# ygtxr1997/CelebBasis

Hardware: NVIDIA H100
Metric: celeb-basis training steps/sec (SD-v1 UNet 512^2, bs=1/GPU) (higher is better)
Workload: dtype f16 operands / f32 accumulate+residual (reference: f32 with TF32 convs)

## Files before the change

### celebbasis_b200/csrc/cb_attention.cu

```cuda
#include <string.h>

#include <type_traits>

#include "cb_common.cuh"

namespace cb {

constexpr int kAttnConsumers = 256;
constexpr int kAttnThreads = kAttnConsumers + 128;
constexpr int kAttnProducerRegs = 24;
constexpr int kAttnConsumerRegs = 240;
constexpr int kBQ = 128;
constexpr int kBKV = 64;

struct AttnParams {
    int nq, nk, heads, images;
    int d;
    int causal;
    int two_pass;
    float scale_log2e;
    void* O;
    long long ldo;
    float* lse;
    void* P;
    long long ldp;
    int is_bf16;
};

template <int DBOX>
struct AttnCfg {
    static constexpr int kQBytes = DBOX * kBQ * 128;
    static constexpr int kKBytes = DBOX * kBKV * 128;
    static constexpr int kVBytes = DBOX * kBKV * 128;
    static constexpr int kPBytes = kBQ * 128;
    static constexpr int kStages = 4;
    static constexpr int kSmemBytes = kQBytes + kStages * (kKBytes + kVBytes) + 2 * kPBytes + 1024 + 256;
};

__device__ __forceinline__ void mbar_wait_consumer(uint32_t bar, uint32_t parity) {
    while (!mbar_try_wait(bar, parity)) {
    }
}

template <uint32_t R>
__device__ __forceinline__ void regs_dealloc() { asm volatile("setmaxnreg.dec.sync.aligned.u32 %0;" ::"n"(R)); }
template <uint32_t R>
__device__ __forceinline__ void regs_alloc() { asm volatile("setmaxnreg.inc.sync.aligned.u32 %0;" ::"n"(R)); }

template <int KS, bool BF16>
__device__ __forceinline__ void mma_rows(float (&acc)[32], uint32_t a, uint32_t a_box, uint32_t b, uint32_t b_box) {
    wgmma_fence();
#pragma unroll
    for (int k = 0; k < KS; ++k)
        Wgmma<64, BF16, 0, 0>::mma(acc, gmma_desc_sw128(a + (k >> 2) * a_box + (k & 3) * 32, 16, 1024),
                                   gmma_desc_sw128(b + (k >> 2) * b_box + (k & 3) * 32, 16, 1024), k > 0 ? 1u : 0u);
    wgmma_commit();
}
template <int KS>
__device__ __forceinline__ void mma_rows_any(bool bf16, float (&acc)[32], uint32_t a, uint32_t a_box, uint32_t b,
                                             uint32_t b_box) {
    if (bf16) mma_rows<KS, true>(acc, a, a_box, b, b_box);
    else mma_rows<KS, false>(acc, a, a_box, b, b_box);
}
template <int NO, bool BF16>
__device__ __forceinline__ void mma_block(float (&acc)[NO / 2], uint32_t a, uint32_t y, uint32_t acc_in) {
    wgmma_fence();
#pragma unroll
    for (int k = 0; k < kBKV / 16; ++k)
        Wgmma<NO, BF16, 0, 1>::mma(acc, gmma_desc_sw128(a + k * 32, 16, 1024), gmma_desc_sw128(y + k * 2048, kBKV * 128, 1024),
                                   k > 0 ? 1u : acc_in);
    wgmma_commit();
}
template <int NO>
__device__ __forceinline__ void mma_block_any(bool bf16, float (&acc)[NO / 2], uint32_t a, uint32_t y, uint32_t acc_in) {
    if (bf16) mma_block<NO, true>(acc, a, y, acc_in);
    else mma_block<NO, false>(acc, a, y, acc_in);
}

__device__ __forceinline__ float fast_exp2(float x) {
    float y;
    asm("ex2.approx.ftz.f32 %0, %1;" : "=f"(y) : "f"(x));
    return y;
}
__device__ __forceinline__ uint32_t pack2(float a, float b, bool bf16) {
    if (bf16) {
        __nv_bfloat162 h = __floats2bfloat162_rn(a, b);
        return *reinterpret_cast<uint32_t*>(&h);
    }
    __half2 h = __floats2half2_rn(a, b);
    return *reinterpret_cast<uint32_t*>(&h);
}
__device__ __forceinline__ void st_a_pair(uint32_t tile, int r, int col, uint32_t v) {
    const uint32_t dst = tile + r * 128 + ((((uint32_t)col >> 3) ^ ((uint32_t)r & 7u)) << 4) + (col & 7) * 2;
    asm volatile("st.shared.b32 [%0], %1;" ::"r"(dst), "r"(v) : "memory");
}
__device__ __forceinline__ float quad_max(float v) {
    v = fmaxf(v, __shfl_xor_sync(0xffffffffu, v, 1));
    return fmaxf(v, __shfl_xor_sync(0xffffffffu, v, 2));
}
__device__ __forceinline__ float quad_sum(float v) {
    v += __shfl_xor_sync(0xffffffffu, v, 1);
    return v + __shfl_xor_sync(0xffffffffu, v, 2);
}

template <int KS>
__global__ void __launch_bounds__(kAttnThreads, 1)
cb_attention_fwd_kernel(const __grid_constant__ CUtensorMap tmQ, const __grid_constant__ CUtensorMap tmK,
                        const __grid_constant__ CUtensorMap tmV, const __grid_constant__ AttnParams p) {
    constexpr int DBOX = (KS + 3) / 4;
    using Cfg = AttnCfg<DBOX>;
    constexpr int kSt = Cfg::kStages;
    constexpr int NO = DBOX * 64;
    extern __shared__ uint8_t smem_raw[];
    const uint32_t base = (smem_u32(smem_raw) + 1023u) & ~1023u;
    const uint32_t sQ = base;
    const uint32_t sKV = sQ + Cfg::kQBytes;
    const uint32_t sP = sKV + kSt * (Cfg::kKBytes + Cfg::kVBytes);
    const uint32_t bars = sP + 2 * Cfg::kPBytes;
    const uint32_t bar_q = bars;
    auto bar_kv_full = [&](int s) { return bars + 8u * (1 + s); };
    auto bar_kv_empty = [&](int s) { return bars + 8u * (1 + kSt + s); };

    const int warp = threadIdx.x >> 5, lane = threadIdx.x & 31;
    const int wg = __shfl_sync(0xffffffffu, warp >> 2, 0);
    const int q0 = blockIdx.x * kBQ;
// ... 659 lines not shown
```

### celebbasis_b200/csrc/cb_common.cuh

```cuda
#pragma once

#include <cuda.h>
#include <cuda_fp16.h>
#include <cuda_bf16.h>
#include <cuda_runtime.h>
#include <stdint.h>

#include "../../include/celebbasis_b200.h"
#include "cb_wgmma.cuh"

namespace cb {

void set_error(const char* fmt, ...);
int  check_cuda(cudaError_t e, const char* what);

#define CB_REQUIRE(cond, code, ...)                      \
    do {                                                 \
        if (!(cond)) {                                   \
            ::cb::set_error(__VA_ARGS__);                \
            return (code);                               \
        }                                                \
    } while (0)

#define CB_CUDA(call)                                                 \
// ... 35 lines not shown
                                                cudaStream_t st, Args&&... args) {
    cudaLaunchConfig_t cfg = {};
    cfg.gridDim = grid;
    cfg.blockDim = block;
    cfg.dynamicSmemBytes = smem;
    cfg.stream = st;
    cudaLaunchAttribute at[2];
    at[0].id = cudaLaunchAttributeClusterDimension;
    at[0].val.clusterDim.x = cluster.x;
    at[0].val.clusterDim.y = cluster.y;
    at[0].val.clusterDim.z = cluster.z;
    at[1].id = cudaLaunchAttributeProgrammaticStreamSerialization;
    at[1].val.programmaticStreamSerializationAllowed = 1;
    cfg.attrs = at;
    cfg.numAttrs = pdl_enabled() ? 2 : 1;
    return cudaLaunchKernelEx(&cfg, kern, static_cast<KArgs>(args)...);
}
#define CB_LAUNCH(kern, grid, block, smem, st, ...) \
    ::cb::launch_kernel(kern, dim3(grid), dim3(block), (size_t)(smem), (st), ##__VA_ARGS__)
#endif

#if defined(__CUDACC__)

__device__ __forceinline__ uint32_t smem_u32(const void* p) {
    return static_cast<uint32_t>(__cvta_generic_to_shared(p));
}

__device__ __forceinline__ uint32_t lane_id() { return threadIdx.x & 31u; }

__device__ __forceinline__ void pdl_launch_dependents() { asm volatile("griddepcontrol.launch_dependents;" ::: "memory"); }
__device__ __forceinline__ void pdl_wait() { asm volatile("griddepcontrol.wait;" ::: "memory"); }
__device__ __forceinline__ void pdl_sync() {
    pdl_launch_dependents();
    pdl_wait();
}

__device__ __forceinline__ bool elect_one() {
    uint32_t pred = 0;
    asm volatile(
        "{\n"
        ".reg .pred P;\n"
        "elect.sync _|P, 0xffffffff;\n"
        "selp.u32 %0, 1, 0, P;\n"
        "}\n"
        : "=r"(pred));
    return pred != 0;
}

__device__ __forceinline__ void mbar_init(uint32_t bar, uint32_t count) {
    asm volatile("mbarrier.init.shared::cta.b64 [%0], %1;" ::"r"(bar), "r"(count));
}
__device__ __forceinline__ void mbar_fence_init() {
    asm volatile("fence.mbarrier_init.release.cluster;" ::: "memory");
}
__device__ __forceinline__ void fence_proxy_async_smem() {
    asm volatile("fence.proxy.async.shared::cta;" ::: "memory");
}
__device__ __forceinline__ void mbar_arrive_expect_tx(uint32_t bar, uint32_t bytes) {
    asm volatile("mbarrier.arrive.expect_tx.shared::cta.b64 _, [%0], %1;" ::"r"(bar), "r"(bytes)
                 : "memory");
}
__device__ __forceinline__ void mbar_arrive(uint32_t bar) {
    asm volatile("mbarrier.arrive.shared::cta.b64 _, [%0];" ::"r"(bar) : "memory");
}
__device__ __forceinline__ bool mbar_try_wait(uint32_t bar, uint32_t parity) {
    uint32_t ok;
    asm volatile(
        "{\n"
        ".reg .pred P;\n"
        "mbarrier.try_wait.parity.shared::cta.b64 P, [%1], %2;\n"
        "selp.u32 %0, 1, 0, P;\n"
        "}\n"
        : "=r"(ok)
        : "r"(bar), "r"(parity)
        : "memory");
    return ok != 0;
}
__device__ __forceinline__ void mbar_wait(uint32_t bar, uint32_t parity) {
    uint32_t spins = 0;
    while (!mbar_try_wait(bar, parity)) {
        if (++spins > (1u << 26)) __trap();
    }
}

__device__ __forceinline__ void tma_prefetch_desc(const CUtensorMap* m) {
    asm volatile("prefetch.tensormap [%0];" ::"l"(reinterpret_cast<uint64_t>(m)) : "memory");
}
__device__ __forceinline__ void tma_load_2d(uint32_t dst, const CUtensorMap* m, uint32_t bar, int c0,
                                            int c1) {
    asm volatile(
        "cp.async.bulk.tensor.2d.shared::cluster.global.mbarrier::complete_tx::bytes [%0], [%1, {%3, %4}], "
        "[%2];" ::"r"(dst),
        "l"(reinterpret_cast<uint64_t>(m)), "r"(bar), "r"(c0), "r"(c1)
        : "memory");
}
__device__ __forceinline__ void tma_load_3d(uint32_t dst, const CUtensorMap* m, uint32_t bar, int c0,
                                            int c1, int c2) {
    asm volatile(
        "cp.async.bulk.tensor.3d.shared::cluster.global.mbarrier::complete_tx::bytes [%0], [%1, {%3, %4, "
        "%5}], [%2];" ::"r"(dst),
        "l"(reinterpret_cast<uint64_t>(m)), "r"(bar), "r"(c0), "r"(c1), "r"(c2)
        : "memory");
}
__device__ __forceinline__ void tma_load_4d(uint32_t dst, const CUtensorMap* m, uint32_t bar, int c0,
                                            int c1, int c2, int c3) {
    asm volatile(
        "cp.async.bulk.tensor.4d.shared::cluster.global.mbarrier::complete_tx::bytes [%0], [%1, {%3, %4, "
        "%5, %6}], [%2];" ::"r"(dst),
        "l"(reinterpret_cast<uint64_t>(m)), "r"(bar), "r"(c0), "r"(c1), "r"(c2), "r"(c3)
        : "memory");
}

__device__ __forceinline__ void tma_bulk_g2s(uint32_t dst, const void* src, uint32_t bytes, uint32_t bar) {
    asm volatile("cp.async.bulk.shared::cluster.global.mbarrier::complete_tx::bytes [%0], [%1], %2, [%3];" ::"r"(dst),
                 "l"(reinterpret_cast<uint64_t>(src)), "r"(bytes), "r"(bar)
                 : "memory");
}

__device__ __forceinline__ void wgmma_fence() { asm volatile("wgmma.fence.sync.aligned;" ::: "memory"); }
__device__ __forceinline__ void wgmma_commit() { asm volatile("wgmma.commit_group.sync.aligned;" ::: "memory"); }
template <int N>
__device__ __forceinline__ void wgmma_wait() { asm volatile("wgmma.wait_group.sync.aligned %0;" ::"n"(N) : "memory"); }
template <int R>
__device__ __forceinline__ void wgmma_fence_regs(float (&d)[R]) {
#pragma unroll
    for (int i = 0; i < R; ++i) asm volatile("" : "+f"(d[i])::"memory");
}
__device__ __forceinline__ void named_bar(int id, int n) { asm volatile("bar.sync %0, %1;" ::"r"(id), "r"(n) : "memory"); }

__device__ __forceinline__ uint32_t cluster_ctarank() {
    uint32_t r;
    asm volatile("mov.u32 %0, %%cluster_ctarank;" : "=r"(r));
    return r;
}
__device__ __forceinline__ void cluster_sync_all() {
    asm volatile("barrier.cluster.arrive.release.aligned;\n\tbarrier.cluster.wait.acquire.aligned;" ::: "memory");
}

__device__ __forceinline__ void st_cluster_f32x8(uint32_t addr, uint32_t cta, const uint32_t* v) {
    asm volatile(
        "{\n"
        ".reg .b32 ra;\n"
        "mapa.shared::cluster.u32 ra, %0, %1;\n"
        "st.shared::cluster.v4.b32 [ra], {%2, %3, %4, %5};\n"
        "st.shared::cluster.v4.b32 [ra + 16], {%6, %7, %8, %9};\n"
        "}\n" ::"r"(addr),
        "r"(cta), "r"(v[0]), "r"(v[1]), "r"(v[2]), "r"(v[3]), "r"(v[4]), "r"(v[5]), "r"(v[6]), "r"(v[7])
        : "memory");
}
__device__ __forceinline__ void st_cluster_f32x2(uint32_t addr, uint32_t cta, float a, float b) {
    asm volatile(
        "{\n"
        ".reg .b32 ra;\n"
        "mapa.shared::cluster.u32 ra, %0, %1;\n"
        "st.shared::cluster.v2.f32 [ra], {%2, %3};\n"
        "}\n" ::"r"(addr),
        "r"(cta), "f"(a), "f"(b)
        : "memory");
}
__device__ __forceinline__ void cluster_arrive_relaxed() { asm volatile("barrier.cluster.arrive.relaxed.aligned;" ::: "memory"); }
__device__ __forceinline__ void cluster_wait() { asm volatile("barrier.cluster.wait.acquire.aligned;" ::: "memory"); }
__device__ __forceinline__ float4 ld_shared_f32x4(uint32_t addr) {
    float4 v;
    asm volatile("ld.shared.v4.f32 {%0, %1, %2, %3}, [%4];" : "=f"(v.x), "=f"(v.y), "=f"(v.z), "=f"(v.w) : "r"(addr) : "memory");
    return v;
}
// ... 43 lines not shown
```

### celebbasis_b200/csrc/cb_gemm.cu

```cuda
#include <algorithm>
#include <stdarg.h>
#include <stdio.h>
#include <stdlib.h>
#include <string.h>

#include "cb_common.cuh"

namespace cb {

constexpr int BM = 128;
constexpr int BK = 64;
constexpr int kThreads = 384;

struct GemmParams {
    int M, N, K;
    int kchunks, taps, kw;
    int ksteps_last;
    int conv;
    int out_h, out_w, img_n;
    int box_w, box_h, box_i;
    int tiles_w, tiles_h;
    int stride, pad_top, pad_left;
    int b_tap_rows, flip_taps;
    void* D;
    int d_dtype;
    long long ldd, d_bs, d_bs2;
    void* D2;
    int d2_dtype;
    long long ldd2;
    int glu;
    const float* act_param;
    const float* d2_scale;
    const float* d2_shift;
    int batch_inner;
    int d_transposed;
    int vec_ok;
    int force_stages;
    const float* bias;
    int bias_row_div;
    long long ldbias;
    const void* R;
    int r_dtype;
    long long ldr, r_bs, r_bs2;
    float alpha;
    int act;
    int bf16;
    unsigned a_bytes, b_bytes;
    int splits, kiters_per_split;
    float* ws;
    unsigned* counters;
    int cluster_sk;
    int dbg_mode;
    unsigned long long* dbg;
};

template <int BN, int kStages>
struct TileCfg {
    static constexpr int kTmemCols = BN <= 64 ? 64 : (BN <= 128 ? 128 : 256);
    static constexpr int kABytes = BM * BK * 2;
    static constexpr int kBBytes = BN * BK * 2;
    static constexpr int kStageBytes = kABytes + kBBytes;
    static constexpr int kSmemBytes = kStages * kStageBytes + 1024 + 256;
    static_assert(kStages * kStageBytes >= BM * (BN + 4) * 4, "the accumulator tile is staged in the TMA ring");
};

__device__ __forceinline__ unsigned long long gtimer() {
    unsigned long long t;
    asm volatile("mov.u64 %0, %globaltimer;" : "=l"(t));
    return t;
}

__device__ __forceinline__ float apply_act(float v, int act) {
    switch (act) {
        case CB_ACT_SILU: return silu_f(v);
        case CB_ACT_GELU: return gelu_f(v);
        case CB_ACT_QUICK_GELU: return quick_gelu_f(v);
        default: return v;
    }
}

__device__ __forceinline__ void apply_act8(float (&f)[8], int act, const float* act_param, int col, int ncols = 8) {
    if (act == CB_ACT_PRELU) {
#pragma unroll
        for (int j = 0; j < 8; ++j)
            if (j < ncols) f[j] = f[j] > 0.f ? f[j] : f[j] * __ldg(act_param + col + j);
    } else {
#pragma unroll
        for (int j = 0; j < 8; ++j) f[j] = apply_act(f[j], act);
    }
}
__device__ __forceinline__ void d2_affine8(float (&g)[8], const float (&f)[8], const float* sc, const float* sh, int col,
                                           int ncols = 8) {
#pragma unroll
    for (int j = 0; j < 8; ++j) g[j] = (sc && j < ncols) ? f[j] * __ldg(sc + col + j) + __ldg(sh + col + j) : f[j];
}

template <typename T>
__device__ __forceinline__ void load8(const T* p, float (&f)[8]);
template <>
__device__ __forceinline__ void load8<__half>(const __half* p, float (&f)[8]) {
    uint4 u = *reinterpret_cast<const uint4*>(p);
    const __half2* h = reinterpret_cast<const __half2*>(&u);
#pragma unroll
    for (int i = 0; i < 4; ++i) {
        float2 t = __half22float2(h[i]);
        f[2 * i] = t.x;
        f[2 * i + 1] = t.y;
    }
}
template <>
__device__ __forceinline__ void load8<__nv_bfloat16>(const __nv_bfloat16* p, float (&f)[8]) {
    uint4 u = *reinterpret_cast<const uint4*>(p);
    const __nv_bfloat162* h = reinterpret_cast<const __nv_bfloat162*>(&u);
#pragma unroll
    for (int i = 0; i < 4; ++i) {
        float2 t = __bfloat1622float2(h[i]);
        f[2 * i] = t.x;
        f[2 * i + 1] = t.y;
    }
}
template <>
__device__ __forceinline__ void load8<float>(const float* p, float (&f)[8]) {
    float4 a = *reinterpret_cast<const float4*>(p);
    float4 b = *reinterpret_cast<const float4*>(p + 4);
    f[0] = a.x; f[1] = a.y; f[2] = a.z; f[3] = a.w;
    f[4] = b.x; f[5] = b.y; f[6] = b.z; f[7] = b.w;
}

template <typename T>
__device__ __forceinline__ void store8(T* p, const float (&f)[8]);
template <>
__device__ __forceinline__ void store8<__half>(__half* p, const float (&f)[8]) {
    uint4 u;
    __half2* h = reinterpret_cast<__half2*>(&u);
#pragma unroll
    for (int i = 0; i < 4; ++i) h[i] = __floats2half2_rn(f[2 * i], f[2 * i + 1]);
    *reinterpret_cast<uint4*>(p) = u;
}
template <>
__device__ __forceinline__ void store8<__nv_bfloat16>(__nv_bfloat16* p, const float (&f)[8]) {
    uint4 u;
    __nv_bfloat162* h = reinterpret_cast<__nv_bfloat162*>(&u);
#pragma unroll
    for (int i = 0; i < 4; ++i) h[i] = __floats2bfloat162_rn(f[2 * i], f[2 * i + 1]);
    *reinterpret_cast<uint4*>(p) = u;
}
template <>
// ... 234 lines not shown
            float f[8] = {0.f, 0.f, 0.f, 0.f, 0.f, 0.f, 0.f, 0.f};
#pragma unroll 4
            for (int s2 = 0; s2 < S; ++s2) {
                const uint32_t a = xbuf + static_cast<uint32_t>(((s2 * GI + gi) * BM + row) * 32);
                const float4 lo = ld_shared_f32x4(a), hi = ld_shared_f32x4(a + 16);
                f[0] += lo.x; f[1] += lo.y; f[2] += lo.z; f[3] += lo.w;
                f[4] += hi.x; f[5] += hi.y; f[6] += hi.z; f[7] += hi.w;
            }
#pragma unroll
            for (int j = 0; j < 8; ++j) f[j] *= p.alpha;
            epilogue_group8<kExt>(p, f, grow, s_brow[row], n0 + g * 8, d_off, r_off, min(8, ncols_tile - g * 8), nullptr,
                                  sbias_of(row, g * 8));
        }
        return;
    }

    if constexpr (kExt) {
        if (p.glu) {
            constexpr int GQ = BN / 16;
#pragma unroll 1
            for (int u = tid; u < BM * GQ; u += kThreads) {
                const int row = u / GQ, q = u % GQ;
                const int vcol = (q >> 2) * 64 + (q & 3) * 8;
                const long long grow = s_grow[row];
                if (vcol >= ncols_tile || grow < 0) continue;
                float fv[8], fg[8];
                stage_ld8(stage + row * kPitch + vcol, p.alpha, fv);
                stage_ld8(stage + row * kPitch + vcol + 32, p.alpha, fg);
#pragma unroll
                for (int j = 0; j < 8; ++j) {
                    fv[j] += p.bias ? s_bias[vcol + j] : 0.f;
                    fg[j] += p.bias ? s_bias[vcol + 32 + j] : 0.f;
                }
                if (p.D) {
                    store8_any(p.D, p.d_dtype, grow * p.ldd + n0 + vcol, fv);
                    store8_any(p.D, p.d_dtype, grow * p.ldd + n0 + vcol + 32, fg);
                }
                float h[8];
#pragma unroll
                for (int j = 0; j < 8; ++j) h[j] = fv[j] * gelu_f(fg[j]);
                store8_any(p.D2, p.d2_dtype, grow * p.ldd2 + ((n0 + (q >> 2) * 64) >> 1) + (q & 3) * 8, h);
            }
            return;
        }
    }

    const bool r_pre = p.R && p.vec_ok && !p.d_transposed;
    uint4 rq[kResAhead + 1][2];
    auto res_fetch = [&](int k, uint4 (&v)[2]) {
        const int u = tid + k * kThreads;
        if (u >= BM * G) return;
        const int row = u / G, col = (u % G) * 8;
        const long long grow = s_grow[row];
        if (grow >= 0 && col + 8 <= ncols_tile) residual_load8(p, r_off + grow * p.ldr + n0 + col, v);
    };
    if (r_pre) {
#pragma unroll
        for (int k = 0; k < kResAhead; ++k) res_fetch(k, rq[k]);
    }
    const int nunits = (BM * G - tid + kThreads - 1) / kThreads;
#pragma unroll 1
    for (int k = 0; k < nunits; ++k) {
        if (r_pre) res_fetch(k + kResAhead, rq[kResAhead]);
        const int u = tid + k * kThreads;
        const int row = p.d_transposed ? u % BM : u / G;
        const int col = (p.d_transposed ? u / BM : u % G) * 8;
        const long long grow = s_grow[row];
        if (col < ncols_tile && grow >= 0) {
            const int ncols = min(8, ncols_tile - col);
            float f[8], r[8];
            stage_ld8(stage + row * kPitch + col, p.alpha, f);
            if (r_pre && ncols == 8) residual_unpack8(p, rq[0], r);
            epilogue_group8<kExt>(p, f, grow, s_brow[row], n0 + col, d_off, r_off, ncols, r_pre && ncols == 8 ? r : nullptr,
                                  sbias_of(row, col));
        }
        if (dbg && k == 0 && tid == 64) dbg[6] = clock64();
        if (r_pre) {
#pragma unroll
            for (int j = 0; j < kResAhead; ++j) { rq[j][0] = rq[j + 1][0]; rq[j][1] = rq[j + 1][1]; }
        }
    }
}

template <int BN, bool A_MN, bool B_MN, int kStages, bool kExt>
__global__ void __launch_bounds__(kThreads, 1)
cb_gemm_kernel(const __grid_constant__ CUtensorMap tmA, const __grid_constant__ CUtensorMap tmB,
               const __grid_constant__ GemmParams p) {
    using Cfg = TileCfg<BN, kStages>;
    using SCfg = StageCfg<BN>;
    extern __shared__ uint8_t smem_raw[];
    const uint32_t smem_base = (smem_u32(smem_raw) + 1023u) & ~1023u;
    float* stage = reinterpret_cast<float*>(smem_raw + (smem_base - smem_u32(smem_raw)));
    const uint32_t bar_base = smem_base + kStages * Cfg::kStageBytes;
    auto full_bar = [&](int s) { return bar_base + 8u * s; };
    auto empty_bar = [&](int s) { return bar_base + 8u * (kStages + s); };

    __shared__ long long s_grow[BM];
    __shared__ int s_brow[BM];
    __shared__ __align__(16) float s_bias[BN];
    const int warp = threadIdx.x >> 5;
    const int wg = __shfl_sync(0xffffffffu, warp >> 2, 0);
    if (p.dbg_mode == 3) { pdl_sync(); return; }
    unsigned long long* dbg = p.dbg ? p.dbg + 8ull * ((blockIdx.z * gridDim.y + blockIdx.y) * gridDim.x + blockIdx.x) : nullptr;
    if (dbg && threadIdx.x == 0) { dbg[0] = clock64(); dbg[7] = gtimer(); }
    const int n0 = blockIdx.x * BN;
    const int m_tile = blockIdx.y;
    const int sp = blockIdx.z % p.splits;
    const int bz = blockIdx.z / p.splits;
    const int zi = bz % p.batch_inner;
    const int zo = bz / p.batch_inner;

    int m0 = 0, ow0 = 0, oh0 = 0, img0 = 0;
    if (p.conv) {
        const int tw = m_tile % p.tiles_w;
        const int th = (m_tile / p.tiles_w) % p.tiles_h;
        const int ti = m_tile / (p.tiles_w * p.tiles_h);
        ow0 = tw * p.box_w;
        oh0 = th * p.box_h;
        img0 = ti * p.box_i;
    } else {
        m0 = m_tile * BM;
    }

    if (threadIdx.x == 0) {
        tma_prefetch_desc(&tmA);
        tma_prefetch_desc(&tmB);
        for (int s = 0; s < kStages; ++s) {
            mbar_init(full_bar(s), 1);
            mbar_init(empty_bar(s), 8);
        }
        mbar_fence_init();
        fence_proxy_async_smem();
    }
    __syncthreads();
    if (dbg && threadIdx.x == 0) dbg[1] = clock64();
    pdl_sync();

    const int kiters_all = p.dbg_mode == 1 ? 0 : p.taps * p.kchunks;
    const int it0 = sp * p.kiters_per_split;
    const int it1 = min(kiters_all, it0 + p.kiters_per_split);

    if (wg == 0) {
        if (threadIdx.x == 0) {
            int s = 0;
            uint32_t ph = 0;
            int tap = it0 / p.kchunks;
            int kc = it0 - tap * p.kchunks;
            int r = tap / p.kw;
            int sx = tap - r * p.kw;
            for (int it = it0; it < it1; ++it) {
                mbar_wait(empty_bar(s), ph ^ 1u);
                mbar_arrive_expect_tx(full_bar(s), p.a_bytes + p.b_bytes);
                const uint32_t a_dst = smem_base + s * Cfg::kStageBytes;
                const uint32_t b_dst = a_dst + Cfg::kABytes;
                const int tap_b = p.flip_taps ? (p.taps - 1 - tap) : tap;
                if (p.conv) {
                    tma_load_4d(a_dst, &tmA, full_bar(s), kc * BK, ow0 * p.stride + sx - p.pad_left,
                                oh0 * p.stride + r - p.pad_top, img0);
                } else if (A_MN) {
                    tma_load_4d(a_dst, &tmA, full_bar(s), m0, kc * BK, zi, zo);
                    tma_load_4d(a_dst + 8192, &tmA, full_bar(s), m0 + 64, kc * BK, zi, zo);
                } else {
                    tma_load_4d(a_dst, &tmA, full_bar(s), kc * BK, m0, zi, zo);
                }
                if (B_MN) {
#pragma unroll
                    for (int j = 0; j < BN / 64; ++j)
                        tma_load_4d(b_dst + j * 8192, &tmB, full_bar(s), n0 + j * 64,
                                    tap_b * p.b_tap_rows + kc * BK, zi, zo);
                } else {
                    tma_load_4d(b_dst, &tmB, full_bar(s), kc * BK, tap_b * p.b_tap_rows + n0, zi, zo);
                }
                if (++s == kStages) { s = 0; ph ^= 1u; }
                if (++kc == p.kchunks) {
                    kc = 0;
                    ++tap;
                    if (++sx == p.kw) { sx = 0; ++r; }
                }
            }
        }
        __syncwarp();
        const int r = threadIdx.x;
        long long grow;
        bool row_valid;
        if (p.conv) {
            const int per_img = p.box_h * p.box_w;
            const int bi = r / per_img;
            const int rem = r - bi * per_img;
            const int bh = rem / p.box_w;
            const int bw = rem - bh * p.box_w;
            const int img = img0 + bi, oh = oh0 + bh, ow = ow0 + bw;
            row_valid = (bi < p.box_i) && (img < p.img_n) && (oh < p.out_h) && (ow < p.out_w);
            grow = ((long long)img * p.out_h + oh) * p.out_w + ow;
        } else {
            grow = m0 + r;
            row_valid = grow < p.M;
        }
        s_grow[r] = row_valid ? grow : -1;
        if (p.bias) {
            const long long tile_row0 = p.conv ? (((long long)img0 * p.out_h + oh0) * p.out_w + ow0) : (long long)m0;
            const long long brow0 = p.bias_row_div > 0 ? tile_row0 / p.bias_row_div : 0;
            const long long brow = p.bias_row_div > 0 ? grow / p.bias_row_div : 0;
            s_brow[r] = brow == brow0 ? -1 : static_cast<int>(brow);
            const int ncols = min(BN, p.N - n0);
            for (int i = r; i < BN; i += 128) s_bias[i] = i < ncols ? p.bias[brow0 * p.ldbias + n0 + i] : 0.f;
        }
    } else {
        float acc[BN / 2];
#pragma unroll
        for (int i = 0; i < BN / 2; ++i) acc[i] = 0.f;
        const uint32_t a_half = static_cast<uint32_t>(wg - 1) * 8192u;
        const bool releaser = (threadIdx.x & 31) == 0;
        int s = 0, s_prev = 0;
        uint32_t ph = 0;
        int kc = it0 % p.kchunks;
        for (int it = it0; it < it1; ++it) {
            mbar_wait(full_bar(s), ph);
            if (dbg && it == it0 && threadIdx.x == 128) dbg[2] = clock64();
            const uint32_t a_src = smem_base + s * Cfg::kStageBytes + a_half;
            const uint32_t b_src = smem_base + s * Cfg::kStageBytes + Cfg::kABytes;
            const int ksteps = (kc == p.kchunks - 1) ? p.ksteps_last : (BK / 16);
            wgmma_fence_regs(acc);
            if (p.bf16) mma_kiter<BN, A_MN, B_MN, true>(acc, a_src, b_src, ksteps);
            else mma_kiter<BN, A_MN, B_MN, false>(acc, a_src, b_src, ksteps);
            wgmma_wait<1>();
            wgmma_fence_regs(acc);
            if (it > it0 && releaser) mbar_arrive(empty_bar(s_prev));
            s_prev = s;
            if (++s == kStages) { s = 0; ph ^= 1u; }
            if (++kc == p.kchunks) kc = 0;
        }
        wgmma_wait<0>();
        wgmma_fence_regs(acc);
        if (it1 > it0 && releaser) mbar_arrive(empty_bar(s_prev));
        if (dbg && threadIdx.x == 128) dbg[3] = clock64();
        named_bar(4, 256);
        const int l = threadIdx.x & 31, w = warp & 3;
        float* srow = stage + ((wg - 1) * 64 + w * 16 + (l >> 2)) * SCfg::kPitch + 2 * (l & 3);
#pragma unroll
        for (int j = 0; j < BN / 8; ++j) {
            *reinterpret_cast<float2*>(srow + 8 * j) = make_float2(acc[4 * j], acc[4 * j + 1]);
            *reinterpret_cast<float2*>(srow + 8 * SCfg::kPitch + 8 * j) = make_float2(acc[4 * j + 2], acc[4 * j + 3]);
        }
    }
    named_bar(2, kThreads);
    const int ncols_tile = min(BN, p.N - n0);
    if (p.splits > 1 && !p.cluster_sk && p.dbg_mode == 0) {
        const unsigned tile_id = (static_cast<unsigned>(bz) * gridDim.y + m_tile) * gridDim.x + blockIdx.x;
        if (!splitk_reduce_to_stage<BN>(p, tile_id, sp, stage, ncols_tile)) return;
    }
    if (p.dbg_mode == 1 || p.dbg_mode == 2) return;
    if (dbg && threadIdx.x == 64) dbg[4] = clock64();
    epilogue_units<BN, kExt>(p, stage, s_grow, s_brow, s_bias, n0, ncols_tile, zo, zi, sp, smem_base + SCfg::kBytes, dbg);
    if (dbg && threadIdx.x == 64) dbg[5] = clock64();
}

typedef CUresult (*EncodeTiledFn)(CUtensorMap*, CUtensorMapDataType, cuuint32_t, void*, const cuuint64_t*,
                                  const cuuint64_t*, const cuuint32_t*, const cuuint32_t*,
                                  CUtensorMapInterleave, CUtensorMapSwizzle, CUtensorMapL2promotion,
                                  CUtensorMapFloatOOBfill);

static EncodeTiledFn get_encode_fn() {
    static EncodeTiledFn fn = nullptr;
    static bool tried = false;
    if (!tried) {
        tried = true;
        void* p = nullptr;
        cudaDriverEntryPointQueryResult q;
        if (cudaGetDriverEntryPoint("cuTensorMapEncodeTiled", &p, cudaEnableDefault, &q) == cudaSuccess &&
            q == cudaDriverEntryPointSuccess) {
            fn = reinterpret_cast<EncodeTiledFn>(p);
        }
    }
    return fn;
}

int make_tmap(CUtensorMap* out, int dtype, int rank, const void* ptr, const uint64_t* dims,
              const uint64_t* strides_bytes , const uint32_t* box, const uint32_t* estr) {
    EncodeTiledFn fn = get_encode_fn();
    CB_REQUIRE(fn != nullptr, CB_ERR_DRIVER, "cuTensorMapEncodeTiled entry point unavailable");
    CB_REQUIRE((reinterpret_cast<uintptr_t>(ptr) & 15u) == 0, CB_ERR_ALIGN, "tensor base %p not 16B aligned", ptr);
    for (int i = 0; i < rank - 1; ++i)
        CB_REQUIRE((strides_bytes[i] & 15u) == 0, CB_ERR_ALIGN, "tensor stride[%d]=%llu bytes not multiple of 16", i,
                   (unsigned long long)strides_bytes[i]);
    CUtensorMapDataType dt = dtype == CB_F16 ? CU_TENSOR_MAP_DATA_TYPE_FLOAT16 : CU_TENSOR_MAP_DATA_TYPE_BFLOAT16;
    CUresult rc = fn(out, dt, (cuuint32_t)rank, const_cast<void*>(ptr), dims, strides_bytes, box, estr,
                     CU_TENSOR_MAP_INTERLEAVE_NONE, CU_TENSOR_MAP_SWIZZLE_128B, CU_TENSOR_MAP_L2_PROMOTION_L2_256B,
                     CU_TENSOR_MAP_FLOAT_OOB_FILL_NONE);
    CB_REQUIRE(rc == CUDA_SUCCESS, CB_ERR_DRIVER,
               "cuTensorMapEncodeTiled failed rc=%d rank=%d dims=[%llu,%llu,%llu,%llu] box=[%u,%u,%u,%u]", (int)rc,
               rank, (unsigned long long)dims[0], (unsigned long long)dims[1],
               (unsigned long long)(rank > 2 ? dims[2] : 0), (unsigned long long)(rank > 3 ? dims[3] : 0), box[0],
               box[1], rank > 2 ? box[2] : 0, rank > 3 ? box[3] : 0);
    return 0;
}

static inline bool needs_ext(const GemmParams& p) { return p.D2 != nullptr || p.act == CB_ACT_PRELU || p.glu; }

template <int BN, bool A_MN, bool B_MN, int kStages, bool kExt>
static int launch_se(const CUtensorMap& tA, const CUtensorMap& tB, const GemmParams& p, dim3 grid, cudaStream_t st) {
    using Cfg = TileCfg<BN, kStages>;
    static bool attr_done = false;
    auto kern = cb_gemm_kernel<BN, A_MN, B_MN, kStages, kExt>;
    if (!attr_done) {
        CB_CUDA(cudaFuncSetAttribute(kern, cudaFuncAttributeMaxDynamicSharedMemorySize, Cfg::kSmemBytes));
        attr_done = true;
    }
    if (p.cluster_sk) {
        const int S = p.splits;
        CB_REQUIRE(S >= 2 && S <= 16 && grid.z % S == 0, CB_ERR_ARG, "cb_gemm(cluster split-K): %d slices not in [2,16]", S);
        static bool np_done = false;
        if (S > 8 && !np_done) {
            CB_CUDA(cudaFuncSetAttribute(kern, cudaFuncAttributeNonPortableClusterSizeAllowed, 1));
            np_done = true;
        }
        CB_CUDA(launch_kernel_cluster(kern, grid, dim3(kThreads), dim3(1, 1, (unsigned)S), (size_t)Cfg::kSmemBytes, st, tA, tB, p));
        CB_CUDA(cudaGetLastError());
        count_launches(1);
        return 0;
    }
CB_LAUNCH((kern), grid, kThreads, Cfg::kSmemBytes, st, tA, tB, p);
    CB_CUDA(cudaGetLastError());
    count_launches(1);
    return 0;
}

template <int BN, bool A_MN, bool B_MN, int kStages>
static int launch_s(const CUtensorMap& tA, const CUtensorMap& tB, const GemmParams& p, dim3 grid, cudaStream_t st) {
    return needs_ext(p) ? launch_se<BN, A_MN, B_MN, kStages, true>(tA, tB, p, grid, st)
                        : launch_se<BN, A_MN, B_MN, kStages, false>(tA, tB, p, grid, st);
}

static int ring_stages(int bn, const GemmParams& p, long long ctas) {
    if (bn == 256) return 4;
    static const int env_force = getenv("CB_GEMM_STAGES") ? atoi(getenv("CB_GEMM_STAGES")) : 0;
    const int force = p.force_stages ? p.force_stages : env_force;
    if (force == 3) return 3;
    if (force == 6 || ctas <= device_sm_count()) return 6;
    return 3;
}
static bool cluster_sk_fits(int bn, int splits, int stages) {
    const long long stage_bytes = ((long long)BM * (bn + 4) * 4 + 1023) / 1024 * 1024;
    const long long ring = (long long)stages * (BM * BK * 2 + bn * BK * 2);
    const long long gi = (bn / 8 + splits - 1) / splits;
    return stage_bytes + (long long)splits * gi * BM * 32 <= ring;
}

template <int BN, bool A_MN, bool B_MN>
static int launch(const CUtensorMap& tA, const CUtensorMap& tB, const GemmParams& p, dim3 grid, cudaStream_t st) {
    if constexpr (BN == 256) {
        return launch_s<BN, A_MN, B_MN, 4>(tA, tB, p, grid, st);
    } else {
        const long long ctas = (long long)grid.x * grid.y * grid.z;
        if (ring_stages(BN, p, ctas) == 6) return launch_s<BN, A_MN, B_MN, 6>(tA, tB, p, grid, st);
        return launch_s<BN, A_MN, B_MN, 3>(tA, tB, p, grid, st);
    }
}

static double tile_time_us(int bn, long long tiles, int kiters, int sms) {
    const double t_iter = (128.0 + bn) * 128.0 / 80e3;
    const long long waves = (tiles + sms - 1) / sms;
    return (double)waves * kiters * t_iter;
}

static int pick_bn(const cb_gemm_desc& d, int m_tiles, int kiters, bool requested = true) {
    const int N = d.N;
    const int sms = device_sm_count();
    int cands[3];
    int nc = 0;
    if (d.b_major == CB_MAJOR_MN) {
        if (N <= 64) return 64;
        cands[nc++] = 128;
        cands[nc++] = 64;
    } else {
        if (N <= 64) return 64;
        cands[nc++] = 160;
        cands[nc++] = 128;
        cands[nc++] = 64;
    }
    static const int env_bn = getenv("CB_GEMM_BN") ? atoi(getenv("CB_GEMM_BN")) : 0;
    const int force_bn = !requested ? 0 : (d.tile_n > 0 ? d.tile_n : env_bn);
    if (force_bn == 256 && N >= 256) return 256;
    for (int i = 0; i < nc; ++i)
        if (cands[i] == force_bn) return force_bn;
    int best = cands[0];
    double best_t = 1e30;
    for (int i = 0; i < nc; ++i) {
        const int bn = cands[i];
        const long long tiles = (long long)ceil_div(N, bn) * m_tiles * d.batch;
        double t = tile_time_us(bn, tiles, kiters, sms) + 0.02 * ceil_div(N, bn);
        if (t < best_t) { best_t = t; best = bn; }
    }
    return best;
}

}

using namespace cb;

extern "C" int cb_gemm(const cb_gemm_desc* dp, void* stream) {
    CB_REQUIRE(dp != nullptr, CB_ERR_ARG, "cb_gemm: null desc");
    const cb_gemm_desc& d = *dp;
    CB_REQUIRE(d.ab_dtype == CB_F16 || d.ab_dtype == CB_BF16, CB_ERR_ARG, "cb_gemm: ab_dtype must be f16/bf16");
    CB_REQUIRE(d.A && d.B && (d.D || (d.glu && d.D2)), CB_ERR_ARG, "cb_gemm: null A/B/D");
    if (d.glu) {
        CB_REQUIRE(d.D2 && d.N % 64 == 0 && d.batch == 1 && !d.d_transposed && !d.R && d.act == CB_ACT_NONE &&
                       d.bias_row_div == 0,
                   CB_ERR_ARG, "cb_gemm(glu): needs D2, N %% 64 == 0, batch 1, no residual / activation / per-image bias");
    }
    CB_REQUIRE(d.N > 0 && d.K > 0 && d.batch > 0, CB_ERR_ARG, "cb_gemm: bad N/K/batch");
    CB_REQUIRE(d.d_dtype >= CB_F16 && d.d_dtype <= CB_F32, CB_ERR_ARG, "cb_gemm: bad d_dtype");
    const int es = 2;
    const bool a_mn = d.a_major == CB_MAJOR_MN, b_mn = d.b_major == CB_MAJOR_MN;
    CB_REQUIRE(!(d.conv && a_mn), CB_ERR_ARG, "cb_gemm: conv mode needs K-major A (NHWC)");
    CB_REQUIRE(!(a_mn && !b_mn), CB_ERR_ARG, "cb_gemm: (A MN-major, B K-major) is not instantiated");

    const int b_in = d.batch_inner > 0 ? d.batch_inner : d.batch;
    CB_REQUIRE(d.batch % b_in == 0, CB_ERR_ARG, "cb_gemm: batch %d not a multiple of batch_inner %d", d.batch, b_in);
    const int b_out = d.batch / b_in;
    GemmParams p;
    memset(&p, 0, sizeof(p));
    p.batch_inner = b_in;
    p.N = d.N;
    p.K = d.K;
    p.kchunks = ceil_div(d.K, BK);
    p.ksteps_last = ceil_div(d.K - (p.kchunks - 1) * BK, 16);
    p.conv = d.conv;
    p.taps = 1;
    p.kw = 1;
    p.b_tap_rows = d.b_tap_rows;
    p.flip_taps = d.flip_taps;

    CUtensorMap tA, tB;
    int m_tiles;
    if (d.conv) {
        CB_REQUIRE(d.img_n > 0 && d.img_h > 0 && d.img_w > 0 && d.out_h > 0 && d.out_w > 0 && d.kh > 0 && d.kw > 0,
                   CB_ERR_ARG, "cb_gemm(conv): bad geometry");
        CB_REQUIRE(d.stride == 1 || d.stride == 2, CB_ERR_ARG, "cb_gemm(conv): stride must be 1 or 2");
        CB_REQUIRE(d.batch == 1, CB_ERR_ARG, "cb_gemm(conv): batch must be 1 (images are rows)");
// ... 50 lines not shown
            uint32_t estr[4] = {1, 1, 1, 1};
            int rc = make_tmap(&tA, d.ab_dtype, 4, d.A, dims, strides, box, estr);
            if (rc) return rc;
        }
    }

    int BN = pick_bn(d, m_tiles, p.taps * p.kchunks);
    if (d.glu && BN % 64 != 0) BN = 128;
    const int b_box_rows = BN;
    p.b_bytes = (unsigned)b_box_rows * BK * es;
    {
        const uint64_t brows_total = (uint64_t)(d.conv ? (int64_t)p.taps * d.b_tap_rows : (b_mn ? d.K : d.N));
        const uint64_t dflt = (uint64_t)(d.ldb * (int64_t)brows_total);
        const uint64_t bs = (uint64_t)(b_in > 1 ? d.b_batch_stride : dflt);
        const uint64_t bs2 = (uint64_t)(b_out > 1 ? d.b_batch_stride2 : dflt);
        uint32_t estr[4] = {1, 1, 1, 1};
        if (b_mn) {
            uint64_t dims[4] = {(uint64_t)d.N, brows_total, (uint64_t)b_in, (uint64_t)b_out};
            uint64_t strides[3] = {(uint64_t)d.ldb * es, bs * es, bs2 * es};
            uint32_t box[4] = {64, BK, 1, 1};
            int rc = make_tmap(&tB, d.ab_dtype, 4, d.B, dims, strides, box, estr);
            if (rc) return rc;
        } else {
            uint64_t dims[4] = {(uint64_t)d.K, brows_total, (uint64_t)b_in, (uint64_t)b_out};
            uint64_t strides[3] = {(uint64_t)d.ldb * es, bs * es, bs2 * es};
            uint32_t box[4] = {BK, (uint32_t)b_box_rows, 1, 1};
            int rc = make_tmap(&tB, d.ab_dtype, 4, d.B, dims, strides, box, estr);
            if (rc) return rc;
        }
    }

    p.D = d.D;
    p.d_dtype = d.d_dtype;
    p.ldd = d.ldd;
    p.d_bs = d.d_batch_stride;
    p.d_bs2 = d.d_batch_stride2;
    p.d_transposed = d.d_transposed;
    p.D2 = d.D2;
    p.d2_dtype = d.d2_dtype;
    p.ldd2 = d.ldd2;
    if (d.D2) {
        CB_REQUIRE(d.batch == 1 && !d.d_transposed, CB_ERR_ARG, "cb_gemm: D2 needs batch == 1 and a non-transposed D");
        CB_REQUIRE(d.d2_dtype >= CB_F16 && d.d2_dtype <= CB_F32, CB_ERR_ARG, "cb_gemm: bad d2_dtype");
        const int es2 = d.d2_dtype == CB_F32 ? 4 : 2;
        CB_REQUIRE((reinterpret_cast<uintptr_t>(d.D2) & 15u) == 0 && (d.ldd2 * es2) % 16 == 0 &&
                       d.ldd2 >= (d.glu ? d.N / 2 : d.N),
                   CB_ERR_ALIGN, "cb_gemm: D2 must be 16-byte aligned with a 16-byte multiple row pitch >= N (N/2 with glu)");
    }
    p.glu = d.glu;
    p.act_param = d.act_param;
    p.d2_scale = d.d2_scale;
    p.d2_shift = d.d2_shift;
    CB_REQUIRE(d.act != CB_ACT_PRELU || d.act_param != nullptr, CB_ERR_ARG, "cb_gemm: CB_ACT_PRELU needs act_param (slopes)");
    CB_REQUIRE((d.d2_scale == nullptr) == (d.d2_shift == nullptr), CB_ERR_ARG, "cb_gemm: d2_scale and d2_shift go together");
    p.bias = d.bias;
    p.bias_row_div = d.bias_row_div;
    p.ldbias = d.ldbias;
    p.R = d.R;
    p.r_dtype = d.r_dtype;
    p.ldr = d.ldr;
    p.r_bs = d.r_batch_stride;
    p.r_bs2 = d.r_batch_stride2;
    p.alpha = d.alpha;
    p.act = d.act;
    p.dbg = reinterpret_cast<unsigned long long*>(d.debug_timeline);
    {
        static const int mode = getenv("CB_GEMM_DBG_MODE") ? atoi(getenv("CB_GEMM_DBG_MODE")) : 0;
        p.dbg_mode = mode;
    }
    p.bf16 = d.ab_dtype == CB_BF16 ? 1 : 0;
    {
        const int des = d.d_dtype == CB_F32 ? 4 : 2;
        bool ok = ((reinterpret_cast<uintptr_t>(d.D) & 15u) == 0) && ((d.ldd * des) % 16 == 0) &&
                  ((d.d_batch_stride * des) % 16 == 0) && ((d.d_batch_stride2 * des) % 16 == 0);
        if (d.R) {
            const int res = d.r_dtype == CB_F32 ? 4 : 2;
            ok = ok && ((reinterpret_cast<uintptr_t>(d.R) & 15u) == 0) && ((d.ldr * res) % 16 == 0) &&
                 ((d.r_batch_stride * res) % 16 == 0) && ((d.r_batch_stride2 * res) % 16 == 0);
        }
        if (d.bias) ok = ok && ((reinterpret_cast<uintptr_t>(d.bias) & 15u) == 0) && ((d.ldbias * 4) % 16 == 0);
        p.vec_ok = ok ? 1 : 0;
    }

    p.force_stages = (d.stages == 3 || d.stages == 6) ? d.stages : 0;
    p.splits = 1;
    p.kiters_per_split = p.taps * p.kchunks;
    {
        const int kiters = p.taps * p.kchunks;
        const int sms = device_sm_count();
        const int bn_s = pick_bn(d, m_tiles, kiters, false);
        const long long tiles_s = (long long)ceil_div(d.N, bn_s) * m_tiles * d.batch;
        const long long counters_bytes = 65536;
        const long long avail = d.splitk_ws_bytes - counters_bytes;
        const long long tiles_max = (long long)ceil_div(d.N, 64) * m_tiles * d.batch;
        const long long slice_bytes = (long long)(d.N + 255) * m_tiles * d.batch * BM * 4;
        if (d.splitk_ws != nullptr && !d.glu && tiles_max <= counters_bytes / 4 &&
            (d.splits > 0 || (tiles_s < sms && kiters >= 8))) {
            const double out_elems = (double)p.M * d.batch * d.N;
            double best_t = tile_time_us(bn_s, tiles_s, kiters, sms);
            int best_sp = 1;
            if (d.splits > 0) {
                best_sp = d.splits < kiters ? d.splits : kiters;
            } else {
                const int max_sp = (int)(sms / tiles_s) < 64 ? (int)(sms / tiles_s) : 64;
                for (int sp = 2; sp <= max_sp; ++sp) {
                    const int per = ceil_div(kiters, sp);
                    if (per < 4) break;
                    const double t = per * ((128.0 + bn_s) * 128.0 / 80e3) + out_elems * sp / 150e3 + 3.0;
                    if (t < best_t) { best_t = t; best_sp = sp; }
                }
            }
            if (best_sp > 1) {
                const int per = ceil_div(kiters, best_sp);
                const int splits = ceil_div(kiters, per);
                if (slice_bytes * splits <= avail) {
                    p.splits = splits;
                    p.kiters_per_split = per;
                    p.counters = reinterpret_cast<unsigned*>(d.splitk_ws);
                    p.ws = reinterpret_cast<float*>(reinterpret_cast<char*>(d.splitk_ws) + counters_bytes);
                }
            }
        }
    }
    cudaStream_t st = reinterpret_cast<cudaStream_t>(stream);
    dim3 grid((unsigned)ceil_div(d.N, BN), (unsigned)m_tiles, (unsigned)(d.batch * p.splits));
    p.cluster_sk = (d.splitk_cluster == 1 && p.splits >= 2 && p.splits <= 16 && p.dbg_mode == 0 &&
                    cluster_sk_fits(BN, p.splits, ring_stages(BN, p, (long long)grid.x * grid.y * grid.z))) ? 1 : 0;
    if (!a_mn && !b_mn) {
        if (BN == 64) return launch<64, false, false>(tA, tB, p, grid, st);
        if (BN == 128) return launch<128, false, false>(tA, tB, p, grid, st);
        if (BN == 256) return launch<256, false, false>(tA, tB, p, grid, st);
        return launch<160, false, false>(tA, tB, p, grid, st);
    } else if (!a_mn && b_mn) {
        if (BN == 64) return launch<64, false, true>(tA, tB, p, grid, st);
        if (BN == 256) return launch<256, false, true>(tA, tB, p, grid, st);
        return launch<128, false, true>(tA, tB, p, grid, st);
    } else {
        if (BN == 64) return launch<64, true, true>(tA, tB, p, grid, st);
        return launch<128, true, true>(tA, tB, p, grid, st);
    }
}
```

Baseline: 56.52.

## Make GEMM pipeline stage count a runtime parameter defaulting to max smem fit

Turns the GEMM TMA ring depth from a template parameter (3/4/6) into a runtime value, defaulting to the largest stage count that fits in shared memory. Previously 3 stages were used whenever the grid exceeded the SM count. The consumer wait also drops the trap-on-timeout spin counter, and two debug modes are added that isolate load-only and MMA-only timing. Deeper rings can hide more load latency but use more shared memory. The 256-column tile still uses 4 stages, and the new debug modes add extra branches in the main loop.

New measurement: 57.32, median of 6. +1.4%, better.

```diff
diff --git a/celebbasis_b200/csrc/cb_attention.cu b/celebbasis_b200/csrc/cb_attention.cu
--- a/celebbasis_b200/csrc/cb_attention.cu
+++ b/celebbasis_b200/csrc/cb_attention.cu
@@ -36,11 +36,6 @@
     static constexpr int kStages = 4;
     static constexpr int kSmemBytes = kQBytes + kStages * (kKBytes + kVBytes) + 2 * kPBytes + 1024 + 256;
 };
-
-__device__ __forceinline__ void mbar_wait_consumer(uint32_t bar, uint32_t parity) {
-    while (!mbar_try_wait(bar, parity)) {
-    }
-}
 
 template <uint32_t R>
 __device__ __forceinline__ void regs_dealloc() { asm volatile("setmaxnreg.dec.sync.aligned.u32 %0;" ::"n"(R)); }
diff --git a/celebbasis_b200/csrc/cb_common.cuh b/celebbasis_b200/csrc/cb_common.cuh
--- a/celebbasis_b200/csrc/cb_common.cuh
+++ b/celebbasis_b200/csrc/cb_common.cuh
@@ -141,6 +141,10 @@
         if (++spins > (1u << 26)) __trap();
     }
 }
+__device__ __forceinline__ void mbar_wait_consumer(uint32_t bar, uint32_t parity) {
+    while (!mbar_try_wait(bar, parity)) {
+    }
+}
 
 __device__ __forceinline__ void tma_prefetch_desc(const CUtensorMap* m) {
     asm volatile("prefetch.tensormap [%0];" ::"l"(reinterpret_cast<uint64_t>(m)) : "memory");
diff --git a/celebbasis_b200/csrc/cb_gemm.cu b/celebbasis_b200/csrc/cb_gemm.cu
--- a/celebbasis_b200/csrc/cb_gemm.cu
+++ b/celebbasis_b200/csrc/cb_gemm.cu
@@ -36,6 +36,7 @@
     int d_transposed;
     int vec_ok;
     int force_stages;
+    int stages;
     const float* bias;
     int bias_row_div;
     long long ldbias;
@@ -54,15 +55,18 @@
     unsigned long long* dbg;
 };
 
-template <int BN, int kStages>
+template <int BN>
 struct TileCfg {
-    static constexpr int kTmemCols = BN <= 64 ? 64 : (BN <= 128 ? 128 : 256);
     static constexpr int kABytes = BM * BK * 2;
     static constexpr int kBBytes = BN * BK * 2;
     static constexpr int kStageBytes = kABytes + kBBytes;
-    static constexpr int kSmemBytes = kStages * kStageBytes + 1024 + 256;
-    static_assert(kStages * kStageBytes >= BM * (BN + 4) * 4, "the accumulator tile is staged in the TMA ring");
+    static constexpr int smem_bytes(int stages) { return stages * kStageBytes + 1024 + 256; }
 };
+constexpr int kDynSmemMax = 227 * 1024 - 2304;
+constexpr int max_stages(int bn) { return (kDynSmemMax - 1024 - 256) / (BM * BK * 2 + bn * BK * 2); }
+constexpr int min_stages(int bn) {
+    return (BM * (bn + 4) * 4 + BM * BK * 2 + bn * BK * 2 - 1) / (BM * BK * 2 + bn * BK * 2);
+}
 
 __device__ __forceinline__ unsigned long long gtimer() {
     unsigned long long t;
@@ -463,15 +467,16 @@
     }
 }
 
-template <int BN, bool A_MN, bool B_MN, int kStages, bool kExt>
+template <int BN, bool A_MN, bool B_MN, bool kExt>
 __global__ void __launch_bounds__(kThreads, 1)
 cb_gemm_kernel(const __grid_constant__ CUtensorMap tmA, const __grid_constant__ CUtensorMap tmB,
                const __grid_constant__ GemmParams p) {
-    using Cfg = TileCfg<BN, kStages>;
+    using Cfg = TileCfg<BN>;
     using SCfg = StageCfg<BN>;
     extern __shared__ uint8_t smem_raw[];
     const uint32_t smem_base = (smem_u32(smem_raw) + 1023u) & ~1023u;
     float* stage = reinterpret_cast<float*>(smem_raw + (smem_base - smem_u32(smem_raw)));
+    const int kStages = p.stages;
     const uint32_t bar_base = smem_base + kStages * Cfg::kStageBytes;
     auto full_bar = [&](int s) { return bar_base + 8u * s; };
     auto empty_bar = [&](int s) { return bar_base + 8u * (kStages + s); };
@@ -520,6 +525,7 @@
     const int kiters_all = p.dbg_mode == 1 ? 0 : p.taps * p.kchunks;
     const int it0 = sp * p.kiters_per_split;
     const int it1 = min(kiters_all, it0 + p.kiters_per_split);
+    const int it_fill = p.dbg_mode == 4 ? min(it1, it0 + kStages) : it1;
 
     if (wg == 0) {
         if (threadIdx.x == 0) {
@@ -529,7 +535,7 @@
             int kc = it0 - tap * p.kchunks;
             int r = tap / p.kw;
             int sx = tap - r * p.kw;
-            for (int it = it0; it < it1; ++it) {
+            for (int it = it0; it < it_fill; ++it) {
                 mbar_wait(empty_bar(s), ph ^ 1u);
                 mbar_arrive_expect_tx(full_bar(s), p.a_bytes + p.b_bytes);
                 const uint32_t a_dst = smem_base + s * Cfg::kStageBytes;
@@ -595,25 +601,30 @@
         int s = 0, s_prev = 0;
         uint32_t ph = 0;
         int kc = it0 % p.kchunks;
+        const bool wait_in_loop = p.dbg_mode != 4, mma_in_loop = p.dbg_mode != 5;
+        if (!wait_in_loop)
+            for (int j = 0; j < it_fill - it0; ++j) mbar_wait_consumer(full_bar(j), 0u);
         for (int it = it0; it < it1; ++it) {
-            mbar_wait(full_bar(s), ph);
+            if (wait_in_loop) mbar_wait_consumer(full_bar(s), ph);
             if (dbg && it == it0 && threadIdx.x == 128) dbg[2] = clock64();
             const uint32_t a_src = smem_base + s * Cfg::kStageBytes + a_half;
             const uint32_t b_src = smem_base + s * Cfg::kStageBytes + Cfg::kABytes;
             const int ksteps = (kc == p.kchunks - 1) ? p.ksteps_last : (BK / 16);
             wgmma_fence_regs(acc);
-            if (p.bf16) mma_kiter<BN, A_MN, B_MN, true>(acc, a_src, b_src, ksteps);
-            else mma_kiter<BN, A_MN, B_MN, false>(acc, a_src, b_src, ksteps);
+            if (mma_in_loop) {
+                if (p.bf16) mma_kiter<BN, A_MN, B_MN, true>(acc, a_src, b_src, ksteps);
+                else mma_kiter<BN, A_MN, B_MN, false>(acc, a_src, b_src, ksteps);
+            }
             wgmma_wait<1>();
             wgmma_fence_regs(acc);
-            if (it > it0 && releaser) mbar_arrive(empty_bar(s_prev));
+            if (it > it0 && releaser && wait_in_loop) mbar_arrive(empty_bar(s_prev));
             s_prev = s;
             if (++s == kStages) { s = 0; ph ^= 1u; }
             if (++kc == p.kchunks) kc = 0;
         }
         wgmma_wait<0>();
         wgmma_fence_regs(acc);
-        if (it1 > it0 && releaser) mbar_arrive(empty_bar(s_prev));
+        if (it1 > it0 && releaser && wait_in_loop) mbar_arrive(empty_bar(s_prev));
         if (dbg && threadIdx.x == 128) dbg[3] = clock64();
         named_bar(4, 256);
         const int l = threadIdx.x & 31, w = warp & 3;
@@ -630,7 +641,7 @@
         const unsigned tile_id = (static_cast<unsigned>(bz) * gridDim.y + m_tile) * gridDim.x + blockIdx.x;
         if (!splitk_reduce_to_stage<BN>(p, tile_id, sp, stage, ncols_tile)) return;
     }
-    if (p.dbg_mode == 1 || p.dbg_mode == 2) return;
+    if (p.dbg_mode == 1 || p.dbg_mode == 2 || p.dbg_mode == 4 || p.dbg_mode == 5) return;
     if (dbg && threadIdx.x == 64) dbg[4] = clock64();
     epilogue_units<BN, kExt>(p, stage, s_grow, s_brow, s_bias, n0, ncols_tile, zo, zi, sp, smem_base + SCfg::kBytes, dbg);
     if (dbg && threadIdx.x == 64) dbg[5] = clock64();
@@ -678,15 +689,16 @@
 
 static inline bool needs_ext(const GemmParams& p) { return p.D2 != nullptr || p.act == CB_ACT_PRELU || p.glu; }
 
-template <int BN, bool A_MN, bool B_MN, int kStages, bool kExt>
+template <int BN, bool A_MN, bool B_MN, bool kExt>
 static int launch_se(const CUtensorMap& tA, const CUtensorMap& tB, const GemmParams& p, dim3 grid, cudaStream_t st) {
-    using Cfg = TileCfg<BN, kStages>;
+    using Cfg = TileCfg<BN>;
     static bool attr_done = false;
-    auto kern = cb_gemm_kernel<BN, A_MN, B_MN, kStages, kExt>;
+    auto kern = cb_gemm_kernel<BN, A_MN, B_MN, kExt>;
     if (!attr_done) {
-        CB_CUDA(cudaFuncSetAttribute(kern, cudaFuncAttributeMaxDynamicSharedMemorySize, Cfg::kSmemBytes));
+        CB_CUDA(cudaFuncSetAttribute(kern, cudaFuncAttributeMaxDynamicSharedMemorySize, Cfg::smem_bytes(max_stages(BN))));
         attr_done = true;
     }
+    const size_t smem = (size_t)Cfg::smem_bytes(p.stages);
     if (p.cluster_sk) {
         const int S = p.splits;
         CB_REQUIRE(S >= 2 && S <= 16 && grid.z % S == 0, CB_ERR_ARG, "cb_gemm(cluster split-K): %d slices not in [2,16]", S);
@@ -695,47 +707,35 @@
             CB_CUDA(cudaFuncSetAttribute(kern, cudaFuncAttributeNonPortableClusterSizeAllowed, 1));
             np_done = true;
         }
-        CB_CUDA(launch_kernel_cluster(kern, grid, dim3(kThreads), dim3(1, 1, (unsigned)S), (size_t)Cfg::kSmemBytes, st, tA, tB, p));
+        CB_CUDA(launch_kernel_cluster(kern, grid, dim3(kThreads), dim3(1, 1, (unsigned)S), smem, st, tA, tB, p));
         CB_CUDA(cudaGetLastError());
         count_launches(1);
         return 0;
     }
-CB_LAUNCH((kern), grid, kThreads, Cfg::kSmemBytes, st, tA, tB, p);
+    CB_LAUNCH((kern), grid, kThreads, smem, st, tA, tB, p);
     CB_CUDA(cudaGetLastError());
     count_launches(1);
     return 0;
 }
 
-template <int BN, bool A_MN, bool B_MN, int kStages>
-static int launch_s(const CUtensorMap& tA, const CUtensorMap& tB, const GemmParams& p, dim3 grid, cudaStream_t st) {
-    return needs_ext(p) ? launch_se<BN, A_MN, B_MN, kStages, true>(tA, tB, p, grid, st)
-                        : launch_se<BN, A_MN, B_MN, kStages, false>(tA, tB, p, grid, st);
-}
-
-static int ring_stages(int bn, const GemmParams& p, long long ctas) {
+template <int BN, bool A_MN, bool B_MN>
+static int launch(const CUtensorMap& tA, const CUtensorMap& tB, const GemmParams& p, dim3 grid, cudaStream_t st) {
+    return needs_ext(p) ? launch_se<BN, A_MN, B_MN, true>(tA, tB, p, grid, st)
+                        : launch_se<BN, A_MN, B_MN, false>(tA, tB, p, grid, st);
+}
+
+static int ring_stages(int bn, const GemmParams& p) {
     if (bn == 256) return 4;
     static const int env_force = getenv("CB_GEMM_STAGES") ? atoi(getenv("CB_GEMM_STAGES")) : 0;
     const int force = p.force_stages ? p.force_stages : env_force;
-    if (force == 3) return 3;
-    if (force == 6 || ctas <= device_sm_count()) return 6;
-    return 3;
+    if (force >= min_stages(bn) && force <= max_stages(bn)) return force;
+    return max_stages(bn);
 }
 static bool cluster_sk_fits(int bn, int splits, int stages) {
     const long long stage_bytes = ((long long)BM * (bn + 4) * 4 + 1023) / 1024 * 1024;
     const long long ring = (long long)stages * (BM * BK * 2 + bn * BK * 2);
     const long long gi = (bn / 8 + splits - 1) / splits;
     return stage_bytes + (long long)splits * gi * BM * 32 <= ring;
-}
-
-template <int BN, bool A_MN, bool B_MN>
-static int launch(const CUtensorMap& tA, const CUtensorMap& tB, const GemmParams& p, dim3 grid, cudaStream_t st) {
-    if constexpr (BN == 256) {
-        return launch_s<BN, A_MN, B_MN, 4>(tA, tB, p, grid, st);
-    } else {
-        const long long ctas = (long long)grid.x * grid.y * grid.z;
-        if (ring_stages(BN, p, ctas) == 6) return launch_s<BN, A_MN, B_MN, 6>(tA, tB, p, grid, st);
-        return launch_s<BN, A_MN, B_MN, 3>(tA, tB, p, grid, st);
-    }
 }
 
 static double tile_time_us(int bn, long long tiles, int kiters, int sms) {
@@ -952,7 +952,7 @@
         p.vec_ok = ok ? 1 : 0;
     }
 
-    p.force_stages = (d.stages == 3 || d.stages == 6) ? d.stages : 0;
+    p.force_stages = d.stages > 0 ? d.stages : 0;
     p.splits = 1;
     p.kiters_per_split = p.taps * p.kchunks;
     {
@@ -994,8 +994,9 @@
     }
     cudaStream_t st = reinterpret_cast<cudaStream_t>(stream);
     dim3 grid((unsigned)ceil_div(d.N, BN), (unsigned)m_tiles, (unsigned)(d.batch * p.splits));
+    p.stages = ring_stages(BN, p);
     p.cluster_sk = (d.splitk_cluster == 1 && p.splits >= 2 && p.splits <= 16 && p.dbg_mode == 0 &&
-                    cluster_sk_fits(BN, p.splits, ring_stages(BN, p, (long long)grid.x * grid.y * grid.z))) ? 1 : 0;
+                    cluster_sk_fits(BN, p.splits, p.stages)) ? 1 : 0;
     if (!a_mn && !b_mn) {
         if (BN == 64) return launch<64, false, false>(tA, tB, p, grid, st);
         if (BN == 128) return launch<128, false, false>(tA, tB, p, grid, st);
```
